# Clemapfel/kmer_index

Measured on AMD Instinct MI355X. Metric: M queries/sec, DNA4 k=10 exact-match batch search, 1e8-bp text, higher is better.
Workload: dtype u32/u64

## Files before the change

kmer_index_amd/csrc/kmx_capi.hip:

```cpp
#include <hip/hip_runtime.h>

#include <algorithm>
#include <atomic>
#include <cstddef>
#include <cstdio>
#include <cstdlib>
#include <cstring>
#include <functional>
#include <memory>
#include <mutex>
#include <string>
#include <system_error>
#include <thread>
#include <utility>
#include <vector>

#include "kmx_approx.h"
#include "kmx_host.h"
#include "kmx_kernels.h"
#include "kmx_vote.h"

namespace {

thread_local std::string g_err;
// ... 355 lines not shown
        void* p = nullptr;
        hipError_t e = hipMalloc(&p, count * sizeof(T) + 64);
        if (e == hipSuccess) { ptrs.push_back(p); *out = static_cast<T*>(p); }
        return e;
    }
};

kmx_status check_device()
{
    int count = 0;
    hipError_t e = hipGetDeviceCount(&count);
    if (e != hipSuccess || count <= 0)
        return fail(KMX_ERR_NO_DEVICE, "no HIP device visible: the kmx engine has no CPU search path");
    return KMX_OK;
}

}

static uint32_t cell_shift_for(uint32_t table_kind, uint64_t n_keys, uint64_t npos, uint64_t region, const kmx_options& o)
{
    if (table_kind != KMX_TABLE_DENSE || o.no_aligned_copy || region > npos) return 0;
    if (const char* e = getenv("KMX_CELLS")) { if (!atoi(e)) return 0; }
    const double c = double(npos) / double(n_keys);
    uint32_t shift = c <= 3.5 ? 3u : c <= 10.5 ? 4u : c <= 24.0 ? 5u : 0u;
    if (const char* e = getenv("KMX_CELL_SHIFT")) { const int v = atoi(e); if (v >= 3 && v <= 5) shift = uint32_t(v); }
    if (!shift) return 0;
    if ((n_keys << shift) > 8 * npos) return 0;
    return shift;
}
static inline uint64_t up32_elems(uint64_t v) { return (v + 31) & ~uint64_t(31); }

static hipError_t publish_headers(kmx_index* ix)
{
    hipError_t e = hipMemcpy(ix->d_index, &ix->h_header, sizeof(KmxIndexDev), hipMemcpyHostToDevice);
    if (e == hipSuccess && ix->d_index_fast) {
        KmxIndexDev hf = ix->h_header;
        if (ix->d_plan_fast) hf.plan = ix->d_plan_fast;
        e = hipMemcpy(ix->d_index_fast, &hf, sizeof hf, hipMemcpyHostToDevice);
    }
    return e;
}
static inline const KmxIndexDev* header_for(const kmx_index* ix, uint32_t flags)
{
    static const bool ref_plan_only = getenv("KMX_REFERENCE_PLAN") != nullptr;
    return ((flags & (KMX_SEARCH_KEEP_MASKS | KMX_SEARCH_REFERENCE_PLAN)) || !ix->d_index_fast || ref_plan_only) ? ix->d_index : ix->d_index_fast;
}

static kmx_status install_images_impl(std::vector<kmx::ElemImage>& images, const uint8_t* tail_kmax, uint64_t n, uint32_t sigma,
                                 uint32_t range, int device, const kmx_options& o, kmx_index** out, void* prebuilt_arena,
                                 uint64_t prebuilt_arena_elems = 0)
{
    auto* ix = new kmx_index();
    ix->device = device;
    ix->n = n;
    ix->sigma = sigma;
    ix->range = range;
    const uint32_t n_ks = uint32_t(images.size());
    uint32_t kmax = 0;
    for (auto& im : images) { ix->ks.push_back(im.k); kmax = std::max(kmax, im.k); }
    kmx_status st = KMX_OK;
    auto bail = [&](kmx_status s) { std::string keep = g_err; kmx_index_free(ix); g_err = keep; return s; };
    for (auto& im : images) {
        if (im.d_offs_prebuilt) ix->allocs.push_back(const_cast<uint32_t*>(im.d_offs_prebuilt));
        if (im.d_atab_prebuilt) ix->allocs.push_back(const_cast<uint32_t*>(im.d_atab_prebuilt));
        if (im.d_ukeys_prebuilt) ix->allocs.push_back(const_cast<uint64_t*>(im.d_ukeys_prebuilt));
        if (im.d_slots_prebuilt) ix->allocs.push_back(const_cast<KmxSlot*>(im.d_slots_prebuilt));
// ... 200 lines not shown
    if (!clone(src->h_header.arena, h.arena_elems * 4 + KMX_ARENA_PAD, 0, &p)) return bail(st);
    h.arena = static_cast<const uint32_t*>(p); ix->d_arena = h.arena;
    if (!clone(src->h_header.tail, h.kmax, 16, &p)) return bail(st);
    h.tail = static_cast<const uint8_t*>(p);
    if (!clone(src->h_header.plan, size_t(h.range) * sizeof(KmxPlanEntry), 16, &p)) return bail(st);
    h.plan = static_cast<const KmxPlanEntry*>(p);
    if (!clone(src->d_plan_fast, src->d_plan_fast ? size_t(h.range) * sizeof(KmxPlanEntry) : 0, 16, &p)) return bail(st);
    ix->d_plan_fast = static_cast<const KmxPlanEntry*>(p);
    {
        void* d = nullptr;
        if (hipMalloc(&d, 16 * 8) == hipSuccess) { (void)hipMemset(d, 0, 16 * 8); ix->allocs.push_back(d); h.dbg = static_cast<unsigned long long*>(d); ix->d_dbg = h.dbg; }
        else { (void)hipGetLastError(); h.dbg = nullptr; }
    }
    for (uint32_t i = 0; i < h.n_ks; ++i) {
        const KmxElemDev& se = src->h_header.elems[i];
        KmxElemDev& de = h.elems[i];
        const auto& sz = src->elem_sizes[i];
        if (!clone(se.offs, sz.n_offs * 4, 16, &p)) return bail(st);
        de.offs = static_cast<const uint32_t*>(p);
        if (!clone(se.atab, sz.n_aoffs * 4, 16, &p)) return bail(st);
        de.atab = static_cast<const uint32_t*>(p);
        if (!clone(se.slots, sz.n_slots * sizeof(KmxSlot), 16, &p)) return bail(st);
        de.slots = static_cast<const KmxSlot*>(p);
        if (!clone(se.ukeys, sz.n_ukeys * 8, 16, &p)) return bail(st);
        de.ukeys = static_cast<const uint64_t*>(p);
        if (!clone(se.dir, se.dir ? (size_t(se.n_dir) + 1) * 4 : 0, 64, &p)) return bail(st);
        de.dir = static_cast<const uint32_t*>(p);
        if (!clone(se.cnt8, se.cnt8 ? size_t(se.n_keys) : 0, 64, &p)) return bail(st);
        de.cnt8 = static_cast<const uint8_t*>(p);
    }
    if (!clone(nullptr, 0, 0, &p)) return bail(st);
    {
        void* d = nullptr;
        e = hipMalloc(&d, sizeof(KmxIndexDev) + 16);
        if (e == hipSuccess) { ix->allocs.push_back(d); e = hipMemcpy(d, &h, sizeof h, hipMemcpyHostToDevice); }
        if (e != hipSuccess) { fail(KMX_ERR_HIP, std::string("replica header: ") + hipGetErrorString(e)); return bail(KMX_ERR_HIP); }
        ix->d_index = static_cast<KmxIndexDev*>(d);
        ix->h_header = h;
        if (ix->d_plan_fast) {
            void* d2 = nullptr;
            e = hipMalloc(&d2, sizeof(KmxIndexDev) + 16);
            if (e == hipSuccess) { ix->allocs.push_back(d2); ix->d_index_fast = static_cast<KmxIndexDev*>(d2); e = publish_headers(ix); }
            if (e != hipSuccess) { fail(KMX_ERR_HIP, std::string("replica header: ") + hipGetErrorString(e)); return bail(KMX_ERR_HIP); }
        }
    }
    *out = ix;
    return KMX_OK;
}

static kmx_status search_finish(kmx_result* r);
static kmx_status add_prefix_levels_impl(kmx_index* ix, const kmx_options& o);
static kmx_status add_prefix_levels(kmx_index* ix, const kmx_options& o)
{
    const kmx::FillVariant keep = ix->fill_variant;
    ix->fill_variant.nt = false;
    const kmx_status st = add_prefix_levels_impl(ix, o);
    ix->fill_variant = keep;
    return st;
}
static kmx_status add_prefix_levels_impl(kmx_index* ix, const kmx_options& o)
{
    int want = o.prefix_levels;
    if (want == 0) {
        want = KMX_DEFAULT_PREFIX_LEVELS;
        if (const char* env = getenv("KMX_PREFIX_LEVELS")) want = atoi(env);
    }
// ... 759 lines not shown

static kmx_status search_device_begin(const kmx_index* cix, const void* d_first, bool nonempty, kmx_result** inout, const char* fn, const char* what,
                                      kmx_index** ix_out)
{
    const std::string f = std::string(fn) + ": ";
    kmx_index* ix = const_cast<kmx_index*>(cix);
    if (ix->broken) return fail(KMX_ERR_HIP, "the index is unusable: a failed kmx_index_extend_query_size_range left its replicas inconsistent");
    if (!ix->peers.empty() && nonempty) {
        hipPointerAttribute_t attr{};
        if (hipPointerGetAttributes(&attr, d_first) != hipSuccess) { (void)hipGetLastError(); return fail(KMX_ERR_INVALID_ARGUMENT, f + what + " is not a device pointer"); }
        kmx_index* pick = nullptr;
        for (size_t i = 0; i < ix->n_replicas() && !pick; ++i)
            if (ix->replica(i)->device == attr.device) pick = ix->replica(i);
        if (!pick) return fail(KMX_ERR_INVALID_ARGUMENT, f + "the queries live on a device that holds no replica of this index");
        ix = pick;
    }
    HIP_TRY(hipSetDevice(ix->device));
    kmx_result* r = *inout;
    if (r && !r->parts.empty()) return fail(KMX_ERR_INVALID_ARGUMENT, f + "the result handle belongs to a multi-device search");
    if (r && r->device != ix->device && r->device_bytes())
        return fail(KMX_ERR_INVALID_ARGUMENT, f + "the result handle holds buffers on another device");
    if (!r) { r = take_result(ix); *inout = r; }
    else KMX_TRY(search_finish(r));
    *ix_out = ix;
    return KMX_OK;
}

static bool scan_hits(kmx_index* ix, kmx_result* r, hipStream_t s, uint64_t tile, uint64_t tile_cap, int items, const kmx::CounterPub& pub)
{
    bool published = false;
    timed(ix, K_SCAN, s, [&] {
        published = kmx::launch_scan_tiles(s, r->cnt.as<uint32_t>(), r->nq, r->bsum.as<uint64_t>(), r->hit_off.as<uint64_t>(),
                                           r->ctr_block(r->ctr_phase) + KMX_CTR_TOTAL_HITS, tile, tile_cap >= 2 ? tile_cap - 1 : 0,
                                           tile_cap >= 2 ? r->tile_q.as<uint32_t>() : nullptr, items, pub);
    });
    return published;
}

using LookupStep = std::function<int(const kmx::QueryDesc&, unsigned long long*, const KmxIndexDev*)>;
static kmx_status search_device_run(kmx_index* ix, kmx_result* r, const uint8_t* qr, const uint64_t* qo, uint64_t nq, uint32_t flags, hipStream_t s,
                                    const LookupStep& lookup)
{
    r->index = ix; r->device = ix->device; r->stream = s;
    (void)hipGetLastError();
    r->flags = flags;
    r->nq = nq;
    r->tally().reset();
    r->host_valid = r->host_masks_valid = false;
    r->small_valid = false;
    r->path = kmx_result::PathRec{};
    r->quiesced = false;
    HIP_TRY(r->ensure_h_ctr());
    HIP_TRY(r->hit_off.ensure((nq + 1) * 8));
    if (nq == 0) {
        HIP_TRY(hipMemsetAsync(r->hit_off.p, 0, 8, s));
        return KMX_OK;
    }
    const std::pair<DevBuf*, size_t> per_query[] = {{&r->src, 8}, {&r->cnt, 4}, {&r->c0, 4}, {&r->aux, 8}, {&r->key, 8}, {&r->p1, 8}, {&r->kind, 1},
                                                    {&r->status, 1}, {&r->stitch_list, 4}, {&r->prefix_list, 4}, {&r->short_list, 4}};
    for (const auto& b : per_query) HIP_TRY(b.first->ensure(nq * b.second));
    HIP_TRY(r->bsum.ensure(std::max(kmx::scan_blocks(nq), kmx::lookup_blocks(nq, 4)) * 8));
    if (r->ctr.cap < 2 * kCtrBytes) {
        HIP_TRY(r->ctr.ensure(2 * kCtrBytes));
        HIP_TRY(hipMemsetAsync(r->ctr.p, 0, 2 * kCtrBytes, s));
        r->ctr_phase = 0;
        r->ctr_clean = true;
    }
// ... 1313 lines not shown
```

kmer_index_amd/csrc/kmx_kernels.h:

```cpp
#pragma once
#include <hip/hip_runtime.h>
#include <stdint.h>
#include "kmx_types.h"


namespace kmx {

struct QueryDesc {
    uint64_t* src;
    uint32_t* cnt;
    uint32_t* c0;
    uint64_t* aux;
    uint64_t* key;
    uint64_t* p1;
    uint8_t* kind;
    uint8_t* status;
    uint32_t* stitch_list;
    uint32_t* prefix_list;
    uint32_t* short_list;
    uint32_t* stitch_hits;
};

uint64_t lookup_blocks(uint64_t nq, int items);
void launch_lookup(hipStream_t s, int items, bool pairs, const KmxIndexDev* ix, const uint8_t* qranks, const uint64_t* qoff,
// ... 11 lines not shown
void launch_small(hipStream_t s, const KmxIndexDev* ix, const uint32_t* arena, unsigned char* mailbox, const KmxSmallLayout& layout, uint32_t n_blocks,
                  const KmxSmallArgs& args, uint32_t nq_total, unsigned long long* xchg, uint32_t flags);
uint64_t scan_blocks(uint64_t n);
void launch_build_dir(hipStream_t s, const uint64_t* d_ukeys, uint64_t n_ukeys, uint32_t shift, uint32_t n_dir, uint32_t* d_dir);
void launch_build_cells(hipStream_t s, const uint32_t* d_offs, const uint32_t* d_region, uint64_t n_keys, uint32_t cell_shift,
                        uint32_t* d_cells, uint8_t* d_cnt8);

struct SparseTables {
    uint64_t* d_ukeys = nullptr;
    uint32_t* d_offs = nullptr;
    KmxSlot* d_slots = nullptr;
    uint64_t n_ukeys = 0;
    uint32_t log2cap = 0;
};
hipError_t sort_kmer_positions(hipStream_t s, const uint8_t* d_text, uint64_t n, uint32_t k, uint32_t sigma, uint32_t key_bits,
                               uint32_t* d_positions);
hipError_t build_sparse_element(hipStream_t s, const uint8_t* d_text, uint64_t n, uint32_t k, uint32_t sigma, uint32_t key_bits,
                                uint32_t* d_positions, SparseTables* out);
hipError_t sort_pairs_u64(hipStream_t s, uint64_t* keys_a, uint32_t* vals_a, uint64_t* keys_b, uint32_t* vals_b, uint64_t n, uint32_t key_bits,
                          bool* in_b);
void launch_scan(hipStream_t s, const uint32_t* in, uint64_t n, uint64_t* bsum, uint64_t* out,
                 unsigned long long* total_out);
struct FillVariant {
    int e;
    bool nt;
};
struct CounterPub {
    const unsigned long long* cur = nullptr;
    unsigned long long* next = nullptr;
    unsigned long long* host = nullptr;
};
bool launch_scan_tiles(hipStream_t s, const uint32_t* in, uint64_t n, uint64_t* bsum, uint64_t* out,
                       unsigned long long* total_out, uint64_t tile, uint64_t n_tiles_cap, uint32_t* tile_q, int lookup_items,
                       const CounterPub& pub = CounterPub());
FillVariant effective_fill_variant(const FillVariant& v, bool rec32);
uint64_t scan_tile();
uint64_t fill_tile(const FillVariant& v);
void launch_partition(hipStream_t s, const uint64_t* off, uint64_t nq, uint64_t tile, uint64_t n_tiles, uint32_t* tile_q);
void launch_fill(hipStream_t s, const FillVariant& v, bool rec32, const KmxIndexDev* ix, const uint32_t* arena, const uint64_t* hit_off,
                 const uint32_t* tile_q, const unsigned long long* total_dev, uint64_t n_tiles, const QueryDesc& d, uint32_t* out);
void launch_compact(hipStream_t s, const uint32_t* arena, const QueryDesc& d, uint64_t n_stitch,
                    const uint64_t* mask_words, const uint64_t* hit_off, uint32_t* out);
void launch_prefix_len(hipStream_t s, const QueryDesc& d, uint64_t n_prefix, const uint32_t* banded, uint32_t* plen);
void launch_build_phase1(hipStream_t s, const uint8_t* d_text, uint64_t n, uint32_t k, uint32_t sigma, uint64_t n_keys,
                         uint32_t* d_hist, uint64_t* d_scratch_u64, uint64_t* d_bsum, uint32_t* d_offs, uint32_t* d_cursor,
                         unsigned int* d_info, unsigned long long* d_total);
void launch_build_phase2(hipStream_t s, const uint8_t* d_text, uint64_t n, uint32_t k, uint32_t sigma, uint64_t n_keys,
                         const uint32_t* d_offs, uint32_t* d_hist, uint64_t* d_scratch_u64, uint64_t* d_bsum, uint32_t* d_cursor,
                         unsigned int* d_info, unsigned long long* d_total, uint32_t* d_region, uint32_t* d_aoffs, uint32_t a0,
                         int sort_mode, uint32_t* d_atab, uint32_t region_end);
void launch_bucket_sort_block(hipStream_t s, const uint32_t* d_offs, uint64_t n_keys, uint32_t* d_positions);
void launch_prefix_sort_small(hipStream_t s, const KmxIndexDev* ix, const uint64_t* qoff, const QueryDesc& d, uint64_t n_prefix,
                              const uint64_t* hit_off, const uint32_t* arena, uint32_t* out);
void launch_prefix_merge_small(hipStream_t s, const KmxIndexDev* ix, const uint64_t* qoff, const QueryDesc& d, uint64_t n_prefix,
                               const uint64_t* hit_off, const uint32_t* arena, uint32_t* out);
struct PrefixSplitRoom {
    void* splits; uint64_t cap_splits;
    void* tiles; uint64_t cap_tiles;
    uint32_t* counters; uint64_t cap_counters;
    uint32_t* scratch; uint64_t cap_scratch;
};
void launch_prefix_bands(hipStream_t s, const KmxIndexDev* ix, const uint64_t* qoff, const QueryDesc& d, uint64_t n_prefix, const uint64_t* hit_off,
                         const uint32_t* arena, uint32_t* banded, void* bands, uint64_t cap_bands, uint32_t* cuts, uint64_t cap_cuts,
                         unsigned long long* used, const PrefixSplitRoom& sr);
void launch_prefix_split(hipStream_t s, const PrefixSplitRoom& sr, const unsigned long long* used, const uint32_t* arena, uint32_t* banded, uint64_t n_text,
                         void* items, uint64_t cap_items, unsigned long long* n_other);
uint64_t prefix_split_bytes(int what);
// ... 20 lines not shown
```

kmer_index_amd/csrc/kmx_kernels.hip:

```cpp
#include <hip/hip_runtime.h>
#include <stdint.h>

#include <algorithm>
#include <atomic>
#include <type_traits>

#include "kmx_kernels.h"

#define KMX_BLOCK 256
#define KMX_WAVE 64
#define KMX_PSORT_PAIR_CAP 512
#ifndef KMX_PSORT_MULTIWAY_RUNS
#define KMX_PSORT_MULTIWAY_RUNS 4
#endif
#define KMX_PM_WAVE_EMAX (((KMX_PSORT_CAP + (KMX_WAVE - KMX_PSORT_MAX_RUNS / 2) - 1) / (KMX_WAVE - KMX_PSORT_MAX_RUNS / 2)) | 1)
#define KMX_PM_WAVE_PAD (KMX_PSORT_MAX_RUNS + KMX_PM_WAVE_EMAX + 5)
#define KMX_PM_TILE 4096
#define KMX_STAGE_CAP 1024
#define KMX_VGROUP 16
#define KMX_VGROUPS (KMX_WAVE / KMX_VGROUP)
#define KMX_VSLICES (64 / KMX_VGROUP)
#define KMX_VSTAGE (1024 / KMX_VGROUPS)
#define KMX_VCH 8

// ... 378 lines not shown
                    kind = KMX_KIND_STITCH; src = r.src; c0 = r.cnt;
                    key = extra.src;
                    p1 = (uint64_t(extra_delta) << 32) | extra.cnt | (nparts > 2 ? KMX_P1_MORE : 0);
                    if (!(flags & KMX_SEARCH_KEEP_MASKS) && stitch_goes_big(r.cnt, extra.cnt)) p1 |= KMX_P1_BIG;
                    if (track) {
                        uint32_t fmask = 0;
                        for (uint32_t t = 0; t < r.cnt; ++t) {
                            const uint32_t b = ar[r.src + t];
#pragma unroll
                            for (uint32_t i = 0; i < KMX_VRESOLVE; ++i) fmask |= uint32_t(((alive >> i) & 1u) && cand[i] == b) << t;
                        }
                        const uint32_t lo = fmask ? uint32_t(__ffs(int(fmask))) - 1u : 0u, len = uint32_t(__popc(fmask));
                        if ((fmask >> lo) == (1u << len) - 1u) {
                            resolved = true;
                            src = r.src + lo;
                            cnt = len;
                        }
                    }
                }
            }
        }
        if (!ranks_ok) { status = KMX_Q_BAD_RANK; kind = KMX_KIND_NONE; cnt = 0; }
    }
    o.src = src; o.aux = aux; o.key = key; o.p1 = p1; o.cnt = cnt; o.c0 = c0; o.kind = kind; o.status = status; o.resolved = resolved;
}

struct BlockCounters {
    unsigned int n_long, base_long;
    unsigned int n_stitch, n_stitch_tiny, n_stitch_short, n_resolved, n_prefix, n_prefix_big, n_prefix_merge, n_prefix_mid, n_prefix_plain, n_error, n_none, n_more;
    unsigned long long words, pelems, hits;
    unsigned int max_runs;
    unsigned int base_stitch, base_stitch_tiny, base_stitch_short, base_prefix, base_prefix_big;
    unsigned long long base_words;
    unsigned int max_fan_exp;
    unsigned int small_keys;
};

template <bool SMALL>
__device__ __forceinline__ bool hash16(const u32x4_a1& w, uint32_t len, uint32_t sigma, uint64_t& h)
{
    uint64_t lo = uint64_t(w[0]) | (uint64_t(w[1]) << 32), hi = uint64_t(w[2]) | (uint64_t(w[3]) << 32);
    {
        const uint32_t sh = (16u - len) * 8u;
        const uint32_t s6 = sh & 63u;
        const uint64_t carry = s6 ? lo >> (64u - s6) : 0;
        const uint64_t hi1 = (hi << s6) | carry, lo1 = lo << s6;
        hi = sh >= 128u ? 0 : sh >= 64u ? lo1 : hi1;
        lo = sh >= 64u ? 0 : lo1;
    }
    const uint32_t wd[4] = {uint32_t(lo), uint32_t(lo >> 32), uint32_t(hi), uint32_t(hi >> 32)};
    uint32_t top = 0;
    if (SMALL) {
        uint32_t acc = 0;
#pragma unroll
        for (uint32_t j = 0; j < 16; ++j) {
            const uint32_t r = (wd[j >> 2] >> (8 * (j & 3))) & 0xFFu;
            top = max(top, r);
            acc = __umul24(acc, sigma) + r;
        }
        h = acc;
    } else {
        uint64_t acc = 0;
#pragma unroll
        for (uint32_t j = 0; j < 16; ++j) {
            const uint32_t r = (wd[j >> 2] >> (8 * (j & 3))) & 0xFFu;
            top = max(top, r);
            acc = acc * sigma + r;
        }
// ... 32 lines not shown
    uint64_t s = slot_hash_dev(h, el->log2cap);
    uint64_t key = uint64_t(pr[0]) | (uint64_t(pr[1]) << 32);
    uint32_t off = pr[2], c = pr[3];
    while (c != 0 && key != h) {
        s = (s + 1) & mask;
        const u64x2 raw = *(const KMX_GLOBAL u64x2*)(slots + s);
        key = raw.x; off = uint32_t(raw.y); c = uint32_t(raw.y >> 32);
    }
    if (c) { r.src = el->arena_base + off; r.cnt = c; }
    return r;
}

#define KMX_PLAN_LDS 256

#ifndef KMX_LOOKUP_OCC
#define KMX_LOOKUP_OCC 4
#endif
template <int ITEMS, bool PAIRS>
__global__ __launch_bounds__(KMX_BLOCK, PAIRS ? KMX_LOOKUP_OCC : (ITEMS > 4 ? 4 : 5)) void k_lookup(const KmxIndexDev* __restrict__ ix,
                                                      const uint8_t* __restrict__ qranks,
                                                      const uint64_t* __restrict__ qoff, uint64_t nq,
                                                      QueryDesc d, unsigned long long* __restrict__ ctr,
                                                      uint64_t* __restrict__ block_hits, uint32_t flags)
{
    __shared__ BlockCounters bc;
    __shared__ KmxElemDev elems_s[KMX_MAX_KS];
    __shared__ uint32_t plan_s[KMX_PLAN_LDS];
    static_assert(KMX_PLAN_LDS == KMX_BLOCK, "one planner entry per thread");
    if (threadIdx.x == 0) {
        bc.n_long = 0;
        bc.n_stitch = bc.n_stitch_tiny = bc.n_stitch_short = bc.n_resolved = bc.n_prefix = bc.n_prefix_big = bc.n_prefix_merge = bc.n_prefix_mid = bc.n_prefix_plain = bc.n_error = bc.n_none = bc.n_more = 0;
        bc.words = bc.pelems = bc.hits = 0;
        bc.max_runs = 0;
        unsigned int j = 0;
        while (j < 63 && ix->pw[j + 1] <= KMX_SUBK_FANOUT_LIMIT) ++j;
        bc.max_fan_exp = j;
        unsigned int small = ix->sigma < (1u << 24) ? 1u : 0u;
        for (uint32_t e = 0; e < ix->n_ks; ++e) {
            const uint64_t nk = ix->elems[e].n_keys;
            if (nk > (uint64_t(1) << 32) || nk / ix->sigma > (uint64_t(1) << 24)) small = 0;
        }
        bc.small_keys = small;
    }
    {
        const uint32_t n_words = ix->n_ks * uint32_t(sizeof(KmxElemDev) / 8);
        const uint64_t* __restrict__ srcw = reinterpret_cast<const uint64_t*>(ix->elems);
        uint64_t* dstw = reinterpret_cast<uint64_t*>(elems_s);
        for (uint32_t i = threadIdx.x; i < n_words; i += KMX_BLOCK) dstw[i] = srcw[i];
        plan_s[threadIdx.x] = threadIdx.x < ix->range ? ((const KMX_GLOBAL uint32_t*)ix->plan)[threadIdx.x] : 0u;
    }
    const uint8_t* __restrict__ qend = qranks + qoff[nq];
    __syncthreads();

    uint8_t kinds[ITEMS];
    unsigned int locs[ITEMS];
    unsigned long long locw[ITEMS];
    bool done[ITEMS];
    uint64_t my_hits = 0;
    const uint32_t sigma = ix->sigma, range = ix->range;
    const bool small_keys = __builtin_amdgcn_readfirstlane(int(bc.small_keys)) != 0;
    const uint8_t* __restrict__ dummy = reinterpret_cast<const uint8_t*>(ix);

    unsigned int my_resolved = 0, my_err = 0, my_none = 0;
    auto emit = [&](int it, uint64_t q, uint8_t kind, uint8_t status, uint64_t src, uint64_t aux, uint64_t key, uint64_t p1, uint32_t cnt,
                    uint32_t c0, bool resolved) {
        unsigned int loc = 0;
        unsigned long long loc_words = 0;
        if (kind == KMX_KIND_STITCH && !resolved) {
            const uint32_t pc = uint32_t(p1);
            if (min(c0, pc) <= KMX_VTINY && max(c0, pc) <= 2 * KMX_VTINY) {
                loc = atomicAdd(&bc.n_stitch_tiny, 1u) | 0x80000000u;
            } else if (!(p1 & (KMX_P1_MORE | KMX_P1_BIG)) && min(c0, pc) <= KMX_VSHORT && max(c0, pc) <= KMX_VSTAGE) {
                loc = atomicAdd(&bc.n_stitch_short, 1u) | 0x40000000u;
                if (pc < c0) p1 |= KMX_P1_SWAP;
            } else {
                if ((p1 & (KMX_P1_MORE | KMX_P1_BIG)) || stitch_is_wide(p1)) atomicAdd(&bc.n_more, 1u);
                loc = atomicAdd(&bc.n_stitch, 1u);
            }
            loc_words = atomicAdd(&bc.words, (unsigned long long)(uint64_t(c0) / 64 + 1));
        }
        if (kind == KMX_KIND_PREFIX) {
            const uint32_t plen = cnt - uint32_t(__popcll(aux));
            if (c0 < 2 || plen < 2) {
                loc = 0xFFFFFFFFu;
                atomicAdd(&bc.n_prefix_plain, 1u);
            } else if (KMX_PSORT_IS_SMALL(c0, plen)) {
                loc = atomicAdd(&bc.n_prefix, 1u);
                if (KMX_PSORT_IS_MERGE(c0, plen)) atomicAdd(&bc.n_prefix_merge, 1u);
            } else {
                loc = atomicAdd(&bc.n_prefix_big, 1u) | 0x80000000u;
                if (plen <= KMX_PSORT_MID_CAP) atomicAdd(&bc.n_prefix_mid, 1u);
                if (plen > KMX_PSORT_BLOCK_CAP) {
                    atomicAdd(&bc.pelems, (unsigned long long)plen);
                    atomicMax(&bc.max_runs, (plen + KMX_PSORT_BLOCK_CAP - 1) / KMX_PSORT_BLOCK_CAP);
                }
            }
        }
        my_resolved += resolved;
        my_err += status != KMX_Q_OK;
        my_none += status == KMX_Q_OK && kind == KMX_KIND_NONE;
        kinds[it] = !resolved ? kind : uint8_t(KMX_KIND_NONE);
        locs[it] = loc;
        locw[it] = loc_words;
        my_hits += cnt;
        d.src[q] = (kind == KMX_KIND_STITCH && !resolved) ? (src | SRC_SLOW) : (kind == KMX_KIND_PREFIX ? (src | SRC_FLAGS) : src);
        d.cnt[q] = cnt;
        d.kind[q] = kind;
        d.status[q] = status;
        if (kind == KMX_KIND_STITCH) {
            if (!resolved) {
                d.c0[q] = c0;
                d.key[q] = key;
                d.p1[q] = p1;
            }
        } else if (kind == KMX_KIND_PREFIX) {
            d.c0[q] = c0;
            d.aux[q] = aux;
            d.key[q] = key;
        }
    };

    uint64_t qb[ITEMS];
    uint32_t qm[ITEMS];
    uint32_t praw[ITEMS];
#pragma unroll
    for (int it = 0; it < ITEMS; ++it) {
        const uint64_t q = (uint64_t(blockIdx.x) * ITEMS + it) * KMX_BLOCK + threadIdx.x;
        const uint64_t qq = q < nq ? q : nq - 1;
        qb[it] = qoff[qq];
        const uint64_t mlen = qoff[qq + 1] - qb[it];
        qm[it] = mlen > 0xFFFFFFFFull ? 0xFFFFFFFFu : uint32_t(mlen);
        kinds[it] = KMX_KIND_NONE;
        locs[it] = 0;
        locw[it] = 0;
    }
#pragma unroll
    for (int it = 0; it < ITEMS; ++it)
        praw[it] = plan_effective(((const KMX_GLOBAL uint32_t*)ix->plan)[min(qm[it], range - 1)]);

    {
        uint32_t eab[ITEMS];
        bool two[ITEMS];
        u32x4_a1 wa[ITEMS], wb[ITEMS];
        unsigned int n_none = 0, n_err = 0;
#pragma unroll
        for (int it = 0; it < ITEMS; ++it) {
            const uint64_t q = (uint64_t(blockIdx.x) * ITEMS + it) * KMX_BLOCK + threadIdx.x;
            const uint32_t m = qm[it], scheme = praw[it] & 0xFF, e = (praw[it] >> 8) & 0xFF;
            const uint32_t kb = elems_s[e].k;
            const bool live = q < nq && m > 0 && m < range;
            const bool one = live && scheme == KMX_SCHEME_SINGLE && kb == m && m <= 16 && qranks + qb[it] + 16 <= qend;
            bool t = false;
            uint32_t ea = e, off = 0;
            if (PAIRS && live && !one && m < KMX_PLAN_LDS) {
                if (scheme == KMX_SCHEME_SINGLE) {
                    const uint32_t rest = m < 2 * kb ? m - kb : 0u;
                    t = m > kb && m <= 2 * kb && kb <= 16 && (rest == 0 || kb - rest <= bc.max_fan_exp);
                    off = m - kb;
                } else if (scheme == KMX_SCHEME_MULTI && ((praw[it] >> 16) & KMX_PLAN_NPARTS_MASK) == 2 && m > kb) {
                    const uint32_t p2 = plan_s[m - kb];
                    ea = (p2 >> 8) & 0xFF;
                    const uint32_t ka = elems_s[ea].k;
                    t = (p2 & 0xFF) != KMX_SCHEME_NONE && ka + kb == m && ka <= 16 && kb <= 16;
                    off = m - kb;
                }
                t = t && qranks + qb[it] + off + 16 <= qend;
            }
            done[it] = one || t;
            two[it] = t;
            eab[it] = ea | (e << 8) | (off << 16);
            wa[it] = *reinterpret_cast<const u32x4_a1*>(done[it] ? qranks + qb[it] : dummy);
            if (PAIRS) wb[it] = *reinterpret_cast<const u32x4_a1*>(t ? qranks + qb[it] + off : dummy);
        }
        uint64_t ha[ITEMS], hb[ITEMS];
        bool oka[ITEMS], okb[ITEMS];
        u32x4_a1 pa[ITEMS], pb[ITEMS];
#pragma unroll
        for (int it = 0; it < ITEMS; ++it) {
            const KmxElemDev* ela = &elems_s[eab[it] & 0xFF];
            const KmxElemDev* elb = &elems_s[(eab[it] >> 8) & 0xFF];
            okb[it] = true; hb[it] = 0;
            if (small_keys) {
                oka[it] = hash16<true>(wa[it], done[it] ? ela->k : 0u, sigma, ha[it]);
                if (PAIRS) okb[it] = hash16<true>(wb[it], two[it] ? elb->k : 0u, sigma, hb[it]);
            } else {
                oka[it] = hash16<false>(wa[it], done[it] ? ela->k : 0u, sigma, ha[it]);
                if (PAIRS) okb[it] = hash16<false>(wb[it], two[it] ? elb->k : 0u, sigma, hb[it]);
            }
            pa[it] = *(const KMX_GLOBAL u32x4_a1*)((done[it] && oka[it]) ? probe_first_addr(ela, ha[it]) : reinterpret_cast<const char*>(dummy));
            if (PAIRS) pb[it] = *(const KMX_GLOBAL u32x4_a1*)((two[it] && okb[it]) ? probe_first_addr(elb, hb[it]) : reinterpret_cast<const char*>(dummy));
// ... 1678 lines not shown
    hipLaunchKernelGGL(k_small, dim3(n_blocks), dim3(KMX_BLOCK), 0, s, ix, arena, mailbox, layout, args, nq_total, xchg, flags);
}

__global__ __launch_bounds__(KMX_BLOCK) void k_scan_reduce(const uint32_t* __restrict__ in, uint64_t n,
                                                           uint64_t* __restrict__ bsum)
{
    const uint64_t base = uint64_t(blockIdx.x) * KMX_SCAN_TILE;
    uint64_t s = 0;
#pragma unroll
    for (int j = 0; j < KMX_SCAN_ITEMS; ++j) {
        uint64_t i = base + uint64_t(j) * KMX_BLOCK + threadIdx.x;
        if (i < n) s += in[i];
    }
    uint64_t total;
    block_exclusive_scan_u64(s, &total);
    if (threadIdx.x == 0) bsum[blockIdx.x] = total;
}

__global__ __launch_bounds__(KMX_BLOCK) void k_scan_spine(uint64_t* __restrict__ bsum, uint64_t nb,
                                                          unsigned long long* __restrict__ total_out)
{
    uint64_t running = 0;
    for (uint64_t base = 0; base < nb; base += KMX_BLOCK) {
        uint64_t i = base + threadIdx.x;
        uint64_t v = i < nb ? bsum[i] : 0;
        uint64_t total;
        uint64_t ex = block_exclusive_scan_u64(v, &total);
        if (i < nb) bsum[i] = running + ex;
        running += total;
    }
    if (threadIdx.x == 0) *total_out = running;
}

template <bool TILES, int SPINE>
__global__ __launch_bounds__(KMX_BLOCK) void k_scan_down(const uint32_t* __restrict__ in, uint64_t n,
                                                         const uint64_t* __restrict__ bsum,
                                                         uint64_t* __restrict__ out, uint64_t tile,
                                                         uint64_t n_tiles_cap, uint32_t* __restrict__ tile_q,
                                                         unsigned long long* __restrict__ total_out, uint64_t n_fine,
                                                         CounterPub pub, uint32_t fine_per_tile)
{
    static_assert(KMX_SCAN_TILE % (KMX_BLOCK * 8) == 0 && KMX_SCAN_TILE % (KMX_BLOCK * 4) == 0, "a scan tile is a whole number of lookup blocks");
    constexpr int ROWS = KMX_SCAN_ITEMS / 4;
    __shared__ uint64_t wave_sum[ROWS][KMX_BLOCK / KMX_WAVE];
    const uint32_t lane = lane_id(), w = threadIdx.x / KMX_WAVE;
    const uint64_t block_base = uint64_t(blockIdx.x) * KMX_SCAN_TILE;
    uint32_t v[ROWS][4];
    uint64_t inc[ROWS];
#pragma unroll
    for (int r = 0; r < ROWS; ++r) {
        const uint64_t i = block_base + uint64_t(r) * (KMX_BLOCK * 4) + uint64_t(threadIdx.x) * 4;
        if (i + 3 < n) {
            const uint4 t = *reinterpret_cast<const uint4*>(in + i);
            v[r][0] = t.x; v[r][1] = t.y; v[r][2] = t.z; v[r][3] = t.w;
        } else {
#pragma unroll
            for (int j = 0; j < 4; ++j) v[r][j] = i + j < n ? in[i + j] : 0u;
        }
        inc[r] = uint64_t(v[r][0]) + v[r][1] + v[r][2] + v[r][3];
    }
    uint64_t own[ROWS];
#pragma unroll
    for (int r = 0; r < ROWS; ++r) own[r] = inc[r];
    for (int off = 1; off < KMX_WAVE; off <<= 1) {
#pragma unroll
        for (int r = 0; r < ROWS; ++r) {
            const uint64_t t = __shfl_up(inc[r], off);
            if (lane >= uint32_t(off)) inc[r] += t;
        }
    }
    if (lane == KMX_WAVE - 1) {
#pragma unroll
        for (int r = 0; r < ROWS; ++r) wave_sum[r][w] = inc[r];
    }
    __syncthreads();
    uint64_t row_base;
    if constexpr (SPINE != 0) {
        __shared__ uint64_t part[KMX_BLOCK / KMX_WAVE];
        const uint64_t mine = SPINE == 2 ? uint64_t(blockIdx.x) * fine_per_tile : uint64_t(blockIdx.x);
        uint64_t acc = 0;
        for (uint64_t i = threadIdx.x; i < mine; i += KMX_BLOCK) acc += bsum[i];
        for (int off = 32; off > 0; off >>= 1) acc += __shfl_xor(acc, off);
        if (lane == 0) part[w] = acc;
        __syncthreads();
        row_base = 0;
#pragma unroll
        for (uint32_t i = 0; i < KMX_BLOCK / KMX_WAVE; ++i) row_base += part[i];
        if (blockIdx.x + 1 == gridDim.x && threadIdx.x == 0) {
            uint64_t own = 0;
            if constexpr (SPINE == 2) { for (uint64_t i = mine; i < n_fine; ++i) own += bsum[i]; }
            else own = bsum[blockIdx.x];
            *total_out = row_base + own;
            if (pub.host) {
#pragma unroll
                for (int c = 0; c < KMX_CTR_COUNT; ++c) {
                    pub.host[c] = c == KMX_CTR_TOTAL_HITS ? row_base + own : pub.cur[c];
                    pub.next[c] = 0;
                }
            }
        }
    } else {
        row_base = bsum[blockIdx.x];
    }
#pragma unroll
    for (int r = 0; r < ROWS; ++r) {
        uint64_t carry = 0, total = 0;
#pragma unroll
        for (uint32_t i = 0; i < KMX_BLOCK / KMX_WAVE; ++i) {
            const uint64_t sw = wave_sum[r][i];
            if (i < w) carry += sw;
// ... 962 lines not shown
        const unsigned int sblocks = (unsigned int)std::min<uint64_t>((sw + 3) / 4, 256 * 16);
        hipLaunchKernelGGL(k_validate_wide, dim3(sblocks ? sblocks : 1), dim3(KMX_VWIDE_BLOCK), 0, s, arena, d, n_stitch, mask_words);
        hipLaunchKernelGGL(k_validate_more_thread, dim3(blocks_for(n_stitch, KMX_BLOCK)), block, 0, s, ix, arena, qranks, qoff, d, n_stitch,
                           uint32_t(n_more >= KMX_VMORE_THREAD_MANY ? KMX_VMORE_THREAD_PARTS_MANY : KMX_VMORE_THREAD_PARTS), mask_words);
        hipLaunchKernelGGL(k_validate_more, grid, block, 0, s, ix, arena, qranks, qoff, d, n_stitch, mask_words);
        const uint64_t wwaves = (n_stitch + KMX_VWAVE_SCAN - 1) / KMX_VWAVE_SCAN;
        const unsigned int wblocks = (unsigned int)std::min<uint64_t>((wwaves + 3) / 4, 256 * 16);
        hipLaunchKernelGGL(k_validate_wave, dim3(wblocks ? wblocks : 1), block, 0, s, ix, arena, qranks, qoff, d, n_stitch, mask_words);
    }
}

uint64_t scan_blocks(uint64_t n) { return blocks_for(n, KMX_SCAN_TILE); }
uint64_t scan_tile() { return KMX_SCAN_TILE; }

#define KMX_SCAN_FUSED_SPINE_BLOCKS 8192

void launch_scan(hipStream_t s, const uint32_t* in, uint64_t n, uint64_t* bsum, uint64_t* out,
                 unsigned long long* total_out)
{
    const unsigned int nb = blocks_for(n, KMX_SCAN_TILE);
    hipLaunchKernelGGL(k_scan_reduce, dim3(nb), dim3(KMX_BLOCK), 0, s, in, n, bsum);
    if (nb <= KMX_SCAN_FUSED_SPINE_BLOCKS) {
        hipLaunchKernelGGL((k_scan_down<false, 1>), dim3(nb), dim3(KMX_BLOCK), 0, s, in, n, bsum, out, uint64_t(1), uint64_t(0),
                           (uint32_t*)nullptr, total_out, uint64_t(0), CounterPub(), 0u);
        return;
    }
    hipLaunchKernelGGL(k_scan_spine, dim3(1), dim3(KMX_BLOCK), 0, s, bsum, uint64_t(nb), total_out);
    hipLaunchKernelGGL((k_scan_down<false, 0>), dim3(nb), dim3(KMX_BLOCK), 0, s, in, n, bsum, out, uint64_t(1), uint64_t(0),
                       (uint32_t*)nullptr, total_out, uint64_t(0), CounterPub(), 0u);
}

bool launch_scan_tiles(hipStream_t s, const uint32_t* in, uint64_t n, uint64_t* bsum, uint64_t* out,
                       unsigned long long* total_out, uint64_t tile, uint64_t n_tiles_cap, uint32_t* tile_q, int lookup_items,
                       const CounterPub& pub)
{
    const unsigned int nb = blocks_for(n, KMX_SCAN_TILE);
    const bool lookup_sums = lookup_items != 0;
    if (lookup_sums && nb <= KMX_SCAN_FUSED_SPINE_BLOCKS) {
        const uint64_t n_fine = lookup_blocks(n, lookup_items);
        const uint32_t fine = uint32_t(KMX_SCAN_TILE / (KMX_BLOCK * lookup_items));
        if (tile_q)
            hipLaunchKernelGGL((k_scan_down<true, 2>), dim3(nb), dim3(KMX_BLOCK), 0, s, in, n, bsum, out, tile, n_tiles_cap, tile_q, total_out, n_fine, pub, fine);
        else
            hipLaunchKernelGGL((k_scan_down<false, 2>), dim3(nb), dim3(KMX_BLOCK), 0, s, in, n, bsum, out, uint64_t(1), uint64_t(0),
                               (uint32_t*)nullptr, total_out, n_fine, pub, fine);
        return pub.host != nullptr;
    }
    if (!tile_q) { launch_scan(s, in, n, bsum, out, total_out); return false; }
    hipLaunchKernelGGL(k_scan_reduce, dim3(nb), dim3(KMX_BLOCK), 0, s, in, n, bsum);
    if (nb <= KMX_SCAN_FUSED_SPINE_BLOCKS) {
        hipLaunchKernelGGL((k_scan_down<true, 1>), dim3(nb), dim3(KMX_BLOCK), 0, s, in, n, bsum, out, tile, n_tiles_cap, tile_q, total_out, uint64_t(0), CounterPub(), 0u);
        return false;
    }
    hipLaunchKernelGGL(k_scan_spine, dim3(1), dim3(KMX_BLOCK), 0, s, bsum, uint64_t(nb), total_out);
    hipLaunchKernelGGL((k_scan_down<true, 0>), dim3(nb), dim3(KMX_BLOCK), 0, s, in, n, bsum, out, tile, n_tiles_cap, tile_q, total_out, uint64_t(0), CounterPub(), 0u);
    return false;
}

uint64_t fill_tile(const FillVariant& v) { return uint64_t(KMX_BLOCK) * v.e; }

void launch_partition(hipStream_t s, const uint64_t* off, uint64_t nq, uint64_t tile, uint64_t n_tiles, uint32_t* tile_q)
{
    hipLaunchKernelGGL(k_partition, dim3(blocks_for(n_tiles + 1, KMX_BLOCK)), dim3(KMX_BLOCK), 0, s, off, nq, tile, n_tiles, tile_q);
}

FillVariant effective_fill_variant(const FillVariant& v, bool rec32)
{
    FillVariant e = v;
    if (!rec32) e.e = 8;
    if (e.e != 4 && e.e != 8 && e.e != 12 && e.e != 16) e.e = 12;
    return e;
}

void launch_fill(hipStream_t s, const FillVariant& v0, bool rec32, const KmxIndexDev* ix, const uint32_t* arena, const uint64_t* hit_off,
// ... 1340 lines not shown
```

kmer_index_amd/csrc/kmx_types.h:

```cpp
#pragma once
#include <stdint.h>
#include "../../include/kmx.h"

#define KMX_MAX_LEVELS 3
#define KMX_DEFAULT_PREFIX_LEVELS 2

struct KmxSlot {
    uint64_t key;
    uint32_t off;
    uint32_t cnt;
};

struct KmxElemDev {
    uint32_t k;
    uint32_t table_kind;
    uint32_t log2cap;
    uint32_t n_ukeys;
    uint64_t n_keys;
    uint64_t arena_base;
    uint64_t npos;
    const uint32_t* offs;
    const KmxSlot* slots;
    const uint64_t* ukeys;
    const uint32_t* atab;
// ... 1 lines not shown
    const uint32_t* dir;
    uint32_t dir_shift;
    uint32_t n_dir;
    const uint8_t* cnt8;
    uint64_t cell_base;
    uint32_t cell_shift;
    uint32_t n_levels;
    uint64_t lvl_offs_at[KMX_MAX_LEVELS];
    uint64_t lvl_base[KMX_MAX_LEVELS];
};

enum { KMX_SCHEME_NONE = 0, KMX_SCHEME_SINGLE = 1, KMX_SCHEME_MULTI = 2, KMX_SCHEME_REPLANNED = 3 };
#define KMX_PLAN_ALT_SHIFT 11
#define KMX_PLAN_NPARTS_MASK ((1u << KMX_PLAN_ALT_SHIFT) - 1u)
struct KmxPlanEntry {
    uint8_t scheme;
    uint8_t elem;
    uint16_t nparts;
};

struct KmxIndexDev {
    uint64_t n;
    uint32_t sigma;
    uint32_t n_ks;
    uint32_t kmax;
    uint32_t range;
    const uint32_t* arena;
    const uint8_t* tail;
    const KmxPlanEntry* plan;
    uint64_t arena_elems;
    unsigned long long* dbg;
    uint64_t pw[64];
    KmxElemDev elems[KMX_MAX_KS];
};

#define KMX_PSORT_IS_SMALL(runs, len) ((len) <= KMX_PSORT_CAP)
#ifndef KMX_PMERGE_MIN_AVG
#define KMX_PMERGE_MIN_AVG 8
#endif
#define KMX_PSORT_IS_MERGE(runs, len)                                                                                   \
    ((len) <= KMX_PSORT_CAP && (runs) >= 2 && (runs) <= KMX_PSORT_MAX_RUNS && !((runs) <= KMX_PMERGE_REG_RUNS && (len) <= KMX_PMERGE_REG_LEN) && \
     (len) >= KMX_PMERGE_MIN_AVG * (runs))
#ifndef KMX_PMERGE_REG_RUNS
#define KMX_PMERGE_REG_RUNS 4
#endif
#ifndef KMX_PMERGE_REG_LEN
#define KMX_PMERGE_REG_LEN 512
#endif
#define KMX_VRESOLVE 4
#define KMX_ARENA_PAD (4096 * 4 + 1024)
#define KMX_VTINY 8
#define KMX_VSHORT 16
#define KMX_PSORT_MAX_RUNS 32
#define KMX_PSORT_CAP 2048
#define KMX_PSORT_BLOCK_CAP 32768
#define KMX_PSORT_MID_CAP 8192

#define KMX_SMALL_NQ 256
#define KMX_SMALL_BLOCKS 32
struct KmxSmallArgs {
    uint16_t nq[KMX_SMALL_BLOCKS];
    uint16_t n_letters[KMX_SMALL_BLOCKS];
};
#define KMX_SMALL_IN_BYTES 8192
#define KMX_SMALL_WCAP 1024
#define KMX_SMALL_WSLOW 32
#define KMX_SMALL_SORT 4096
// ... 61 lines not shown
```

Measured before the change: 7090.

## Precompute header constants on host, read plan from LDS, fuse spine sum into scan

Moves the per-block computation of max_fan_exp and small_keys from the lookup kernel into host-side header setup, so each block reads them instead of looping over pw and elements. The lookup kernel now loads query offsets earlier and reads plan entries from the shared-memory copy when every query length fits, avoiding global plan reads. A new scan variant (SPINE==3) computes each block's prefix from the fine block sums with a vectorised unrolled reduction, and has the last block publish the total and counters. It adds header fields and more complex scan code paths.

```diff
diff --git a/kmer_index_amd/csrc/kmx_capi.hip b/kmer_index_amd/csrc/kmx_capi.hip
--- a/kmer_index_amd/csrc/kmx_capi.hip
+++ b/kmer_index_amd/csrc/kmx_capi.hip
@@ -411,6 +411,7 @@
 
 static hipError_t publish_headers(kmx_index* ix)
 {
+    kmx_header_constants(&ix->h_header);
     hipError_t e = hipMemcpy(ix->d_index, &ix->h_header, sizeof(KmxIndexDev), hipMemcpyHostToDevice);
     if (e == hipSuccess && ix->d_index_fast) {
         KmxIndexDev hf = ix->h_header;
@@ -677,6 +678,7 @@
     if (!clone(nullptr, 0, 0, &p)) return bail(st);
     {
         void* d = nullptr;
+        kmx_header_constants(&h);
         e = hipMalloc(&d, sizeof(KmxIndexDev) + 16);
         if (e == hipSuccess) { ix->allocs.push_back(d); e = hipMemcpy(d, &h, sizeof h, hipMemcpyHostToDevice); }
         if (e != hipSuccess) { fail(KMX_ERR_HIP, std::string("replica header: ") + hipGetErrorString(e)); return bail(KMX_ERR_HIP); }
@@ -1502,7 +1504,7 @@
     timed(ix, K_SCAN, s, [&] {
         published = kmx::launch_scan_tiles(s, r->cnt.as<uint32_t>(), r->nq, r->bsum.as<uint64_t>(), r->hit_off.as<uint64_t>(),
                                            r->ctr_block(r->ctr_phase) + KMX_CTR_TOTAL_HITS, tile, tile_cap >= 2 ? tile_cap - 1 : 0,
-                                           tile_cap >= 2 ? r->tile_q.as<uint32_t>() : nullptr, items, pub);
+                                           tile_cap >= 2 ? r->tile_q.as<uint32_t>() : nullptr, items, pub, items != 0 && !r->windows);
     });
     return published;
 }
diff --git a/kmer_index_amd/csrc/kmx_kernels.h b/kmer_index_amd/csrc/kmx_kernels.h
--- a/kmer_index_amd/csrc/kmx_kernels.h
+++ b/kmer_index_amd/csrc/kmx_kernels.h
@@ -67,7 +67,7 @@
 };
 bool launch_scan_tiles(hipStream_t s, const uint32_t* in, uint64_t n, uint64_t* bsum, uint64_t* out,
                        unsigned long long* total_out, uint64_t tile, uint64_t n_tiles_cap, uint32_t* tile_q, int lookup_items,
-                       const CounterPub& pub = CounterPub());
+                       const CounterPub& pub = CounterPub(), bool front = false);
 FillVariant effective_fill_variant(const FillVariant& v, bool rec32);
 uint64_t scan_tile();
 uint64_t fill_tile(const FillVariant& v);
diff --git a/kmer_index_amd/csrc/kmx_kernels.hip b/kmer_index_amd/csrc/kmx_kernels.hip
--- a/kmer_index_amd/csrc/kmx_kernels.hip
+++ b/kmer_index_amd/csrc/kmx_kernels.hip
@@ -434,8 +434,6 @@
     unsigned int max_runs;
     unsigned int base_stitch, base_stitch_tiny, base_stitch_short, base_prefix, base_prefix_big;
     unsigned long long base_words;
-    unsigned int max_fan_exp;
-    unsigned int small_keys;
 };
 
 template <bool SMALL>
@@ -534,15 +532,16 @@
         bc.n_stitch = bc.n_stitch_tiny = bc.n_stitch_short = bc.n_resolved = bc.n_prefix = bc.n_prefix_big = bc.n_prefix_merge = bc.n_prefix_mid = bc.n_prefix_plain = bc.n_error = bc.n_none = bc.n_more = 0;
         bc.words = bc.pelems = bc.hits = 0;
         bc.max_runs = 0;
-        unsigned int j = 0;
-        while (j < 63 && ix->pw[j + 1] <= KMX_SUBK_FANOUT_LIMIT) ++j;
-        bc.max_fan_exp = j;
-        unsigned int small = ix->sigma < (1u << 24) ? 1u : 0u;
-        for (uint32_t e = 0; e < ix->n_ks; ++e) {
-            const uint64_t nk = ix->elems[e].n_keys;
-            if (nk > (uint64_t(1) << 32) || nk / ix->sigma > (uint64_t(1) << 24)) small = 0;
-        }
-        bc.small_keys = small;
+    }
+    uint64_t qb[ITEMS];
+    uint32_t qm[ITEMS];
+#pragma unroll
+    for (int it = 0; it < ITEMS; ++it) {
+        const uint64_t q = (uint64_t(blockIdx.x) * ITEMS + it) * KMX_BLOCK + threadIdx.x;
+        const uint64_t qq = q < nq ? q : nq - 1;
+        qb[it] = qoff[qq];
+        const uint64_t mlen = qoff[qq + 1] - qb[it];
+        qm[it] = mlen > 0xFFFFFFFFull ? 0xFFFFFFFFu : uint32_t(mlen);
     }
     {
         const uint32_t n_words = ix->n_ks * uint32_t(sizeof(KmxElemDev) / 8);
@@ -560,7 +559,8 @@
     bool done[ITEMS];
     uint64_t my_hits = 0;
     const uint32_t sigma = ix->sigma, range = ix->range;
-    const bool small_keys = __builtin_amdgcn_readfirstlane(int(bc.small_keys)) != 0;
+    const bool small_keys = ix->small_keys != 0;
+    const uint32_t max_fan_exp = ix->max_fan_exp;
     const uint8_t* __restrict__ dummy = reinterpret_cast<const uint8_t*>(ix);
 
     unsigned int my_resolved = 0, my_err = 0, my_none = 0;
@@ -622,23 +622,25 @@
         }
     };
 
-    uint64_t qb[ITEMS];
-    uint32_t qm[ITEMS];
     uint32_t praw[ITEMS];
 #pragma unroll
     for (int it = 0; it < ITEMS; ++it) {
-        const uint64_t q = (uint64_t(blockIdx.x) * ITEMS + it) * KMX_BLOCK + threadIdx.x;
-        const uint64_t qq = q < nq ? q : nq - 1;
-        qb[it] = qoff[qq];
-        const uint64_t mlen = qoff[qq + 1] - qb[it];
-        qm[it] = mlen > 0xFFFFFFFFull ? 0xFFFFFFFFu : uint32_t(mlen);
         kinds[it] = KMX_KIND_NONE;
         locs[it] = 0;
         locw[it] = 0;
     }
-#pragma unroll
-    for (int it = 0; it < ITEMS; ++it)
-        praw[it] = plan_effective(((const KMX_GLOBAL uint32_t*)ix->plan)[min(qm[it], range - 1)]);
+    {
+        bool beyond = false;
+#pragma unroll
+        for (int it = 0; it < ITEMS; ++it) beyond = beyond || qm[it] >= KMX_PLAN_LDS;
+        if (beyond) {
+#pragma unroll
+            for (int it = 0; it < ITEMS; ++it) praw[it] = plan_effective(((const KMX_GLOBAL uint32_t*)ix->plan)[min(qm[it], range - 1)]);
+        } else {
+#pragma unroll
+            for (int it = 0; it < ITEMS; ++it) praw[it] = plan_effective(plan_s[qm[it]]);
+        }
+    }
 
     {
         uint32_t eab[ITEMS];
@@ -657,7 +659,7 @@
             if (PAIRS && live && !one && m < KMX_PLAN_LDS) {
                 if (scheme == KMX_SCHEME_SINGLE) {
                     const uint32_t rest = m < 2 * kb ? m - kb : 0u;
-                    t = m > kb && m <= 2 * kb && kb <= 16 && (rest == 0 || kb - rest <= bc.max_fan_exp);
+                    t = m > kb && m <= 2 * kb && kb <= 16 && (rest == 0 || kb - rest <= max_fan_exp);
                     off = m - kb;
                 } else if (scheme == KMX_SCHEME_MULTI && ((praw[it] >> 16) & KMX_PLAN_NPARTS_MASK) == 2 && m > kb) {
                     const uint32_t p2 = plan_s[m - kb];
@@ -2402,6 +2404,43 @@
     if (threadIdx.x == 0) *total_out = running;
 }
 
+#define KMX_SPINE_UNROLL 4
+#define KMX_SPINE_STEP (2 * KMX_SPINE_UNROLL * KMX_BLOCK)
+__device__ __forceinline__ uint64_t spine_partial(const uint64_t* __restrict__ bsum, uint64_t count)
+{
+    typedef uint64_t u64x2s __attribute__((ext_vector_type(2)));
+    uint64_t acc[KMX_SPINE_UNROLL];
+#pragma unroll
+    for (int u = 0; u < KMX_SPINE_UNROLL; ++u) acc[u] = 0;
+    if (!count) return 0;
+    const uint64_t head = (reinterpret_cast<uintptr_t>(bsum) & 8u) ? 1u : 0u;
+    const u64x2s* __restrict__ pairs = reinterpret_cast<const u64x2s*>(bsum + head);
+    const uint64_t n_pairs = (count - head) / 2;
+    const bool odd = ((count - head) & 1u) != 0;
+    uint64_t single = 0;
+    if (threadIdx.x == 0) single = (head ? bsum[0] : 0) + (odd ? bsum[count - 1] : 0);
+    uint64_t p = threadIdx.x;
+    for (; p + uint64_t(KMX_SPINE_UNROLL - 1) * KMX_BLOCK < n_pairs; p += uint64_t(KMX_SPINE_UNROLL) * KMX_BLOCK) {
+        u64x2s x[KMX_SPINE_UNROLL];
+#pragma unroll
+        for (int u = 0; u < KMX_SPINE_UNROLL; ++u) x[u] = pairs[p + uint64_t(u) * KMX_BLOCK];
+        __builtin_amdgcn_sched_barrier(0);
+#pragma unroll
+        for (int u = 0; u < KMX_SPINE_UNROLL; ++u) acc[u] += x[u][0] + x[u][1];
+    }
+    if (n_pairs) {
+        u64x2s x[KMX_SPINE_UNROLL];
+#pragma unroll
+        for (int u = 0; u < KMX_SPINE_UNROLL; ++u) x[u] = pairs[min(p + uint64_t(u) * KMX_BLOCK, n_pairs - 1)];
+#pragma unroll
+        for (int u = 0; u < KMX_SPINE_UNROLL; ++u) acc[u] += p + uint64_t(u) * KMX_BLOCK < n_pairs ? x[u][0] + x[u][1] : 0;
+    }
+    uint64_t s = single;
+#pragma unroll
+    for (int u = 0; u < KMX_SPINE_UNROLL; ++u) s += acc[u];
+    return s;
+}
+
 template <bool TILES, int SPINE>
 __global__ __launch_bounds__(KMX_BLOCK) void k_scan_down(const uint32_t* __restrict__ in, uint64_t n,
                                                          const uint64_t* __restrict__ bsum,
@@ -2411,23 +2450,57 @@
                                                          CounterPub pub, uint32_t fine_per_tile)
 {
     static_assert(KMX_SCAN_TILE % (KMX_BLOCK * 8) == 0 && KMX_SCAN_TILE % (KMX_BLOCK * 4) == 0, "a scan tile is a whole number of lookup blocks");
+    constexpr bool FRONT = SPINE == 3;
     constexpr int ROWS = KMX_SCAN_ITEMS / 4;
     __shared__ uint64_t wave_sum[ROWS][KMX_BLOCK / KMX_WAVE];
     const uint32_t lane = lane_id(), w = threadIdx.x / KMX_WAVE;
     const uint64_t block_base = uint64_t(blockIdx.x) * KMX_SCAN_TILE;
     uint32_t v[ROWS][4];
     uint64_t inc[ROWS];
-#pragma unroll
-    for (int r = 0; r < ROWS; ++r) {
-        const uint64_t i = block_base + uint64_t(r) * (KMX_BLOCK * 4) + uint64_t(threadIdx.x) * 4;
-        if (i + 3 < n) {
-            const uint4 t = *reinterpret_cast<const uint4*>(in + i);
-            v[r][0] = t.x; v[r][1] = t.y; v[r][2] = t.z; v[r][3] = t.w;
+    uint64_t acc = 0, own_sum = 0, ctr_cur = 0;
+    if constexpr (FRONT) {
+        if (block_base + KMX_SCAN_TILE <= n) {
+            uint4 t[ROWS];
+#pragma unroll
+            for (int r = 0; r < ROWS; ++r)
+                t[r] = *reinterpret_cast<const uint4*>(in + block_base + uint64_t(r) * (KMX_BLOCK * 4) + uint64_t(threadIdx.x) * 4);
+#pragma unroll
+            for (int r = 0; r < ROWS; ++r) { v[r][0] = t[r].x; v[r][1] = t[r].y; v[r][2] = t[r].z; v[r][3] = t[r].w; }
         } else {
 #pragma unroll
-            for (int j = 0; j < 4; ++j) v[r][j] = i + j < n ? in[i + j] : 0u;
-        }
-        inc[r] = uint64_t(v[r][0]) + v[r][1] + v[r][2] + v[r][3];
+            for (int r = 0; r < ROWS; ++r) {
+                const uint64_t i = block_base + uint64_t(r) * (KMX_BLOCK * 4) + uint64_t(threadIdx.x) * 4;
+                if (i + 3 < n) {
+                    const uint4 t = *reinterpret_cast<const uint4*>(in + i);
+                    v[r][0] = t.x; v[r][1] = t.y; v[r][2] = t.z; v[r][3] = t.w;
+                } else {
+#pragma unroll
+                    for (int j = 0; j < 4; ++j) v[r][j] = i + j < n ? in[i + j] : 0u;
+                }
+            }
+        }
+        static_assert(KMX_CTR_COUNT <= KMX_WAVE && KMX_SCAN_TILE / (KMX_BLOCK * 4) <= KMX_WAVE, "a lane per counter / per own sum");
+        const uint64_t mine = uint64_t(blockIdx.x) * fine_per_tile;
+        acc = spine_partial(bsum, mine);
+        if (blockIdx.x + 1 == gridDim.x && w == 0) {
+            if (mine + lane < n_fine) own_sum = bsum[mine + lane];
+            if (pub.host && lane < KMX_CTR_COUNT) ctr_cur = pub.cur[lane];
+        }
+#pragma unroll
+        for (int r = 0; r < ROWS; ++r) inc[r] = uint64_t(v[r][0]) + v[r][1] + v[r][2] + v[r][3];
+    } else {
+#pragma unroll
+        for (int r = 0; r < ROWS; ++r) {
+            const uint64_t i = block_base + uint64_t(r) * (KMX_BLOCK * 4) + uint64_t(threadIdx.x) * 4;
+            if (i + 3 < n) {
+                const uint4 t = *reinterpret_cast<const uint4*>(in + i);
+                v[r][0] = t.x; v[r][1] = t.y; v[r][2] = t.z; v[r][3] = t.w;
+            } else {
+#pragma unroll
+                for (int j = 0; j < 4; ++j) v[r][j] = i + j < n ? in[i + j] : 0u;
+            }
+            inc[r] = uint64_t(v[r][0]) + v[r][1] + v[r][2] + v[r][3];
+        }
     }
     uint64_t own[ROWS];
 #pragma unroll
@@ -2445,7 +2518,24 @@
     }
     __syncthreads();
     uint64_t row_base;
-    if constexpr (SPINE != 0) {
+    if constexpr (FRONT) {
+        __shared__ uint64_t part[KMX_BLOCK / KMX_WAVE];
+        for (int off = 32; off > 0; off >>= 1) acc += __shfl_xor(acc, off);
+        if (lane == 0) part[w] = acc;
+        __syncthreads();
+        row_base = 0;
+#pragma unroll
+        for (uint32_t i = 0; i < KMX_BLOCK / KMX_WAVE; ++i) row_base += part[i];
+        if (blockIdx.x + 1 == gridDim.x && w == 0) {
+            for (int off = 32; off > 0; off >>= 1) own_sum += __shfl_xor(own_sum, off);
+            const uint64_t grand = row_base + own_sum;
+            if (lane == 0) *total_out = grand;
+            if (pub.host && lane < KMX_CTR_COUNT) {
+                pub.host[lane] = lane == KMX_CTR_TOTAL_HITS ? grand : ctr_cur;
+                pub.next[lane] = 0;
+            }
+        }
+    } else if constexpr (SPINE != 0) {
         __shared__ uint64_t part[KMX_BLOCK / KMX_WAVE];
         const uint64_t mine = SPINE == 2 ? uint64_t(blockIdx.x) * fine_per_tile : uint64_t(blockIdx.x);
         uint64_t acc = 0;
@@ -3474,14 +3564,20 @@
 
 bool launch_scan_tiles(hipStream_t s, const uint32_t* in, uint64_t n, uint64_t* bsum, uint64_t* out,
                        unsigned long long* total_out, uint64_t tile, uint64_t n_tiles_cap, uint32_t* tile_q, int lookup_items,
-                       const CounterPub& pub)
+                       const CounterPub& pub, bool front)
 {
     const unsigned int nb = blocks_for(n, KMX_SCAN_TILE);
     const bool lookup_sums = lookup_items != 0;
     if (lookup_sums && nb <= KMX_SCAN_FUSED_SPINE_BLOCKS) {
         const uint64_t n_fine = lookup_blocks(n, lookup_items);
         const uint32_t fine = uint32_t(KMX_SCAN_TILE / (KMX_BLOCK * lookup_items));
-        if (tile_q)
+        if (front) {
+            if (tile_q)
+                hipLaunchKernelGGL((k_scan_down<true, 3>), dim3(nb), dim3(KMX_BLOCK), 0, s, in, n, bsum, out, tile, n_tiles_cap, tile_q, total_out, n_fine, pub, fine);
+            else
+                hipLaunchKernelGGL((k_scan_down<false, 3>), dim3(nb), dim3(KMX_BLOCK), 0, s, in, n, bsum, out, uint64_t(1), uint64_t(0),
+                                   (uint32_t*)nullptr, total_out, n_fine, pub, fine);
+        } else if (tile_q)
             hipLaunchKernelGGL((k_scan_down<true, 2>), dim3(nb), dim3(KMX_BLOCK), 0, s, in, n, bsum, out, tile, n_tiles_cap, tile_q, total_out, n_fine, pub, fine);
         else
             hipLaunchKernelGGL((k_scan_down<false, 2>), dim3(nb), dim3(KMX_BLOCK), 0, s, in, n, bsum, out, uint64_t(1), uint64_t(0),
diff --git a/kmer_index_amd/csrc/kmx_types.h b/kmer_index_amd/csrc/kmx_types.h
--- a/kmer_index_amd/csrc/kmx_types.h
+++ b/kmer_index_amd/csrc/kmx_types.h
@@ -57,7 +57,21 @@
     unsigned long long* dbg;
     uint64_t pw[64];
     KmxElemDev elems[KMX_MAX_KS];
+    uint32_t max_fan_exp;
+    uint32_t small_keys;
 };
+static inline void kmx_header_constants(KmxIndexDev* h)
+{
+    uint32_t j = 0;
+    while (j < 63 && h->pw[j + 1] <= KMX_SUBK_FANOUT_LIMIT) ++j;
+    h->max_fan_exp = j;
+    uint32_t small = h->sigma < (1u << 24) ? 1u : 0u;
+    for (uint32_t e = 0; e < h->n_ks && h->sigma; ++e) {
+        const uint64_t nk = h->elems[e].n_keys;
+        if (nk > (uint64_t(1) << 32) || nk / h->sigma > (uint64_t(1) << 24)) small = 0;
+    }
+    h->small_keys = small;
+}
 
 #define KMX_PSORT_IS_SMALL(runs, len) ((len) <= KMX_PSORT_CAP)
 #ifndef KMX_PMERGE_MIN_AVG
```

New measurement: 7121, median of 6. Within noise of the previous version (+0.4%).
